# tkkiran/Robust-Conditional-GAN

Measured on AMD Instinct MI355X. Metric: images/sec G+D train step (CIFAR-10 RCGAN bs=64), higher is better.
Workload: dtype bf16

## Files before the change

include/rcgan_hip.h:

```cpp
#ifndef RCGAN_HIP_H
#define RCGAN_HIP_H

#include <stddef.h>
#include <stdint.h>

#ifdef __cplusplus
extern "C" {
#endif

#define RCGAN_OK 0
#define RCGAN_EINVALID_ARG (-1)
#define RCGAN_EUNSUPPORTED_SHAPE (-2)
#define RCGAN_EWORKSPACE_TOO_SMALL (-3)
#define RCGAN_EHIP (-4)
#define RCGAN_ERCCL (-5)

#define RCGAN_F32 0
#define RCGAN_BF16 1
#define RCGAN_F16 2

#define RCGAN_ACT_NONE 0
#define RCGAN_ACT_RELU 1
#define RCGAN_ACT_LRELU 2
#define RCGAN_ACT_TANH 3
// ... 137 lines not shown
int rcgan_bn_bwd(rcgan_ctx* ctx, int n, int rows_per_sample, int c, int n_labels, int dtype,
                 const void* x, const void* y, const void* dy, const int32_t* labels,
                 const float* gamma, const float* mean, const float* rstd, int act,
                 void* dx, int accumulate_dx, float* dgamma, float* dbeta, int accumulate, void* ws, size_t ws_bytes);
int rcgan_bn_bwd2(rcgan_ctx* ctx, int n, int rows_per_sample, int c, int n_labels, int dtype, const void* x, const void* y,
                  const void* dy, const int32_t* labels, const float* gamma, const float* beta, const float* mean, const float* rstd,
                  int act, void* dx, int accumulate_dx, float* dgamma, float* dbeta, int accumulate, void* ws, size_t ws_bytes);
int rcgan_bn_infer(rcgan_ctx* ctx, int rows, int c, int dtype, const void* x, const float* gamma,
                   const float* beta, const float* moving_mean, const float* moving_var, float eps,
                   int act, void* y);
int rcgan_bn_infer_bwd(rcgan_ctx* ctx, int rows, int c, int dtype, const void* y, const void* dy, const float* gamma,
                       const float* moving_var, float eps, int act, void* dx, int accumulate);

typedef struct rcgan_sn_item {
  const float* w;
  float* u;
  float* sigma;
  float* save;
  int k, c, update;
} rcgan_sn_item;
size_t rcgan_sn_save_floats(int k, int c);
int rcgan_sn_power_iter(rcgan_ctx* ctx, const rcgan_sn_item* items, int n_items);
typedef struct rcgan_sn_bwd_item {
  const float* w; const float* dwbar; float* dw; float* save ; int k, c, accumulate;
} rcgan_sn_bwd_item;
int rcgan_sn_bwd(rcgan_ctx* ctx, const rcgan_sn_bwd_item* items, int n_items);
typedef struct rcgan_sn_adam {
  float* w; float* g; float* m; float* v; size_t count;
  float* hyper;
  float beta1, beta2, eps, clip, grad_scale;
  int n_ranges; const size_t* ranges;
} rcgan_sn_adam;
int rcgan_sn_bwd_adam(rcgan_ctx* ctx, const rcgan_sn_bwd_item* items, int n_items, const rcgan_sn_adam* opt);

int rcgan_act_fwd(rcgan_ctx* ctx, size_t count, int dtype, int act, const void* x, void* y);
int rcgan_act_bwd(rcgan_ctx* ctx, size_t count, int dtype, int act, const void* x_or_y, const void* dy,
                  void* dx, int accumulate);
int rcgan_add(rcgan_ctx* ctx, size_t count, int dtype, const void* a, const void* b, void* y);
int rcgan_axpby(rcgan_ctx* ctx, size_t count, int dtype, float alpha, const void* a, float beta, void* y);
int rcgan_cast(rcgan_ctx* ctx, size_t count, int src_dtype, const void* src, int dst_dtype, void* dst);
int rcgan_meanpool2_fwd(rcgan_ctx* ctx, int n, int h, int w, int c, int dtype, const void* x, void* y);
int rcgan_meanpool2_bwd(rcgan_ctx* ctx, int n, int h, int w, int c, int dtype, const void* dy, void* dx, int accumulate);
int rcgan_upsample2_fwd(rcgan_ctx* ctx, int n, int h, int w, int c, int dtype, const void* x, void* y);
int rcgan_upsample2_bwd(rcgan_ctx* ctx, int n, int h, int w, int c, int dtype, const void* dy, void* dx, int accumulate);
int rcgan_pad_channels(rcgan_ctx* ctx, size_t rows, int c, int before, int after, int dtype, const void* x, void* y);
int rcgan_concat_channels_fwd(rcgan_ctx* ctx, int n, int hw, int c1, int c2, int dtype, const void* x,
                              const float* yb, void* y);
int rcgan_concat_channels_bwd(rcgan_ctx* ctx, int n, int hw, int c1, int c2, int dtype, const void* dy, void* dx);
int rcgan_tile_rows_fwd(rcgan_ctx* ctx, size_t count, int reps, int dtype, const void* x, void* y);
int rcgan_tile_rows_bwd(rcgan_ctx* ctx, size_t count, int reps, int dtype, const void* dy, void* dx, int accumulate);
int rcgan_transpose_f32(rcgan_ctx* ctx, int rows, int cols, const float* x, float* y, int accumulate);
int rcgan_preprocess_cifar(rcgan_ctx* ctx, int n, const int32_t* images_chw, const float* noise_chw,
                           int dtype, void* y_nhwc);

int rcgan_rng_fill(rcgan_ctx* ctx, size_t count, int dtype, int kind, float lo, float hi, uint64_t seed,
                   void* state, void* y);

int rcgan_act_meanhw_fwd(rcgan_ctx* ctx, int n, int hw, int c, int dtype, int act, const void* x, float* feat);
int rcgan_act_meanhw_bwd(rcgan_ctx* ctx, int n, int hw, int c, int dtype, int act, const void* x,
                         const float* dfeat, void* dx);
int rcgan_gather_rows(rcgan_ctx* ctx, int n, int d, const float* table, const int32_t* idx, float* out);
int rcgan_scatter_add_rows(rcgan_ctx* ctx, int n, int d, int v, const float* src, const int32_t* idx,
                           float* table_grad, int accumulate);
int rcgan_proj_logit_fwd(rcgan_ctx* ctx, int n, int d, const float* feat, const float* psi, const float* emb,
                         float* logit);
int rcgan_proj_logit_bwd(rcgan_ctx* ctx, int n, int d, const float* feat, const float* emb, const float* dlogit,
// ... 114 lines not shown
```

robust-conditional-gan_amd/_lib.py:

```python
import ctypes as C
import os

_HERE = os.path.dirname(os.path.abspath(__file__))
LIB_PATH = os.environ.get("RCGAN_LIB_PATH") or os.path.join(_HERE, "librcgan_hip.so")
LIB_PATH_F16 = os.environ.get("RCGAN_LIB_PATH_F16") or os.path.join(_HERE, "librcgan_hip_f16.so")

F32, BF16, F16 = 0, 1, 2
ACT_NONE, ACT_RELU, ACT_LRELU, ACT_TANH, ACT_SIGMOID = 0, 1, 2, 3, 4
CONV_IN_UPSAMPLE2X, CONV_IN_RELU, CONV_ACCUMULATE, CONV_FORCE_DIRECT, CONV_OUT_MEANPOOL2, CONV_RESID_UPSAMPLE2X = 1, 2, 4, 8, 16, 32
LOSS_HINGE_REAL, LOSS_HINGE_FAKE, LOSS_NEG_MEAN, LOSS_CE_ONES, LOSS_CE_ZEROS = 0, 1, 2, 3, 4
QUERY_TR_READ = 0
F32_PRECISION_HIGHEST, F32_PRECISION_HIGH = 0, 1
F32_PRECISIONS = {"highest": F32_PRECISION_HIGHEST, "high": F32_PRECISION_HIGH}

RCGAN_EHIP, RCGAN_ERCCL = -4, -5
EINVALID_ARG, EUNSUPPORTED_SHAPE = -1, -2
ERRORS = {-1: "RCGAN_EINVALID_ARG", -2: "RCGAN_EUNSUPPORTED_SHAPE", -3: "RCGAN_EWORKSPACE_TOO_SMALL",
          -4: "RCGAN_EHIP", -5: "RCGAN_ERCCL"}


def source_hash():
    import glob
    import hashlib
    h = hashlib.sha256()
# ... 109 lines not shown
    "rcgan_conv2d_fwd_bn": (I, [P, DP, P, P, P, P, I, P, P, P, P, P, I]),
    "rcgan_conv2d_fwd_bn_residual": (I, [P, DP, P, P, P, P, P, I, P, P, P, P, P, I]),
    "rcgan_conv_fused_pool_ok": (I, [DP]),
    "rcgan_conv_resid_up_ok": (I, [DP]),
    "rcgan_conv_wgrad_pool_ok": (I, [DP]),
    "rcgan_conv2d_fwd_residual": (I, [P, DP, P, P, P, P, P]),
    "rcgan_conv2d_bwd_data": (I, [P, DP, P, P, P, P, P, SZ]),
    "rcgan_conv2d_bwd_data_residual": (I, [P, DP, P, P, P, P, P, P, SZ]),
    "rcgan_conv2d_bwd_weight": (I, [P, DP, P, P, P, P, I, P, SZ]),
    "rcgan_conv2d_bwd_weight_group": (I, [P, I, P, P, P, P, P, I, P, SZ]),
    "rcgan_deconv2d_fwd": (I, [P, DP, P, P, P, P]),
    "rcgan_deconv2d_bwd_data": (I, [P, DP, P, P, P]),
    "rcgan_deconv2d_bwd_data_cols": (I, [P, DP, P, P, P, I]),
    "rcgan_deconv2d_bwd_weight": (I, [P, DP, P, P, P, P, I, P, SZ]),
    "rcgan_deconv2d_bwd_weight_concat_bytes": (SZ, [DP, I]),
    "rcgan_deconv2d_bwd_weight_concat": (I, [P, DP, P, P, I, P, P, P, I, P, SZ]),
    "rcgan_linear_fwd": (I, [P, I, I, I, I, P, P, P, P, P]),
    "rcgan_linear_bwd_data": (I, [P, I, I, I, I, P, P, P, P, I]),
    "rcgan_linear_bwd_weight": (I, [P, I, I, I, I, P, P, P, P, I, P, SZ]),
    "rcgan_linear_workspace_bytes": (SZ, [I, I, I]),
    "rcgan_bn_workspace_bytes": (SZ, [I, I]),
    "rcgan_bn_workspace_bytes_labels": (SZ, [I, I, I]),
    "rcgan_bn_stats": (I, [P, I, I, I, P, F, P, P, P, P, F, P, SZ]),
    "rcgan_bn_apply_fwd": (I, [P, I, I, I, I, I, P, P, P, P, P, P, I, P, P, SZ]),
    "rcgan_bn_fwd_segments": (I, [P, I, I, I, I, I, I, P, P, P, P, F, I, P, P, P, P, SZ]),
    "rcgan_bn_bwd": (I, [P, I, I, I, I, I, P, P, P, P, P, P, P, I, P, I, P, P, I, P, SZ]),
    "rcgan_bn_bwd2": (I, [P, I, I, I, I, I, P, P, P, P, P, P, P, P, I, P, I, P, P, I, P, SZ]),
    "rcgan_bn_infer": (I, [P, I, I, I, P, P, P, P, P, F, I, P]),
    "rcgan_bn_infer_bwd": (I, [P, I, I, I, P, P, P, P, F, I, P, I]),
    "rcgan_sn_save_floats": (SZ, [I, I]),
    "rcgan_sn_power_iter": (I, [P, C.POINTER(SnItem), I]),
    "rcgan_sn_bwd": (I, [P, C.POINTER(SnBwdItem), I]),
    "rcgan_sn_bwd_adam": (I, [P, C.POINTER(SnBwdItem), I, C.POINTER(SnAdam)]),
    "rcgan_act_fwd": (I, [P, SZ, I, I, P, P]),
    "rcgan_act_bwd": (I, [P, SZ, I, I, P, P, P, I]),
    "rcgan_add": (I, [P, SZ, I, P, P, P]),
    "rcgan_axpby": (I, [P, SZ, I, F, P, F, P]),
    "rcgan_cast": (I, [P, SZ, I, P, I, P]),
    "rcgan_meanpool2_fwd": (I, [P, I, I, I, I, I, P, P]),
    "rcgan_meanpool2_bwd": (I, [P, I, I, I, I, I, P, P, I]),
    "rcgan_upsample2_fwd": (I, [P, I, I, I, I, I, P, P]),
    "rcgan_upsample2_bwd": (I, [P, I, I, I, I, I, P, P, I]),
    "rcgan_pad_channels": (I, [P, SZ, I, I, I, I, P, P]),
    "rcgan_concat_channels_fwd": (I, [P, I, I, I, I, I, P, P, P]),
    "rcgan_concat_channels_bwd": (I, [P, I, I, I, I, I, P, P]),
    "rcgan_tile_rows_fwd": (I, [P, SZ, I, I, P, P]),
    "rcgan_tile_rows_bwd": (I, [P, SZ, I, I, P, P, I]),
    "rcgan_transpose_f32": (I, [P, I, I, P, P, I]),
    "rcgan_preprocess_cifar": (I, [P, I, P, P, I, P]),
    "rcgan_rng_fill": (I, [P, SZ, I, I, F, F, C.c_uint64, P, P]),
    "rcgan_act_meanhw_fwd": (I, [P, I, I, I, I, I, P, P]),
    "rcgan_act_meanhw_bwd": (I, [P, I, I, I, I, I, P, P, P]),
    "rcgan_gather_rows": (I, [P, I, I, P, P, P]),
    "rcgan_scatter_add_rows": (I, [P, I, I, I, P, P, P, I]),
    "rcgan_proj_logit_fwd": (I, [P, I, I, P, P, P, P]),
    "rcgan_proj_logit_bwd": (I, [P, I, I, P, P, P, P, P, P, I]),
    "rcgan_proj_logit_all_fwd": (I, [P, I, I, I, P, P, P, P]),
    "rcgan_proj_logit_all_bwd": (I, [P, I, I, I, P, P, P, P, P, P, I]),
    "rcgan_loss_fwd_bwd": (I, [P, I, I, I, P, P, F, P, P, P]),
    "rcgan_bce_onehot_fwd_bwd": (I, [P, I, I, P, P, F, P, P]),
    "rcgan_dtrunk": (I, [P, I, I, P, P, P, P, P]),
    "rcgan_dtrunk_pooled": (I, [P, I, I, P, P, P, P, P, P, P, P]),
    "rcgan_dtrunk_prepare": (I, [P, P, P]),
    "rcgan_conv_rf_ok": (I, [C.POINTER(ConvDesc)]),
    "rcgan_conv_rf_fragment_bytes": (SZ, [C.POINTER(ConvDesc)]),
    "rcgan_conv_rf_prepare": (I, [P, I, C.POINTER(ConvDesc), P, P]),
# ... 70 lines not shown
```

robust-conditional-gan_amd/cifar.py:

```python
import ctypes as C
import os

import warnings

import numpy as np
import torch

from . import _lib as L
from . import ops as O
from .ops_cifar import NO_OPS, Conv2D, Linear, cond_batchnorm, embed_y, spectral_normed_weight
from .runtime import DT, Context, ParamGroup, check_f32_matmul_precision
from .variables import Graph, scoped, variable_scope

Z_DIM = 128
DIM_G = 128
DIM_D = 128
VOCAB_SIZE = 10
EMBEDDING_DIM = 300
IMG_SIZE = 32
IMG_DIM = 3
OUTPUT_DIM = 3072
N_CRITIC = 5
GEN_BS_MULTIPLE = 2
ALGORITHMS = ("rcgan", "rcgan-u", "biased", "unbiased")
# ... 874 lines not shown
            self.PD.version += 1
            return
        self._optimise_or_publish(steps)

    def _critic_graph_ok(self):
        return (self.critic_graph and self.fused_tail and self._fakes_left == N_CRITIC and self._rides_inputs() and self._slice_mirror == 0)

    def critic_steps(self, batches, iteration=None):
        it = self.iteration if iteration is None else iteration
        packed = isinstance(batches, torch.Tensor)
        assert (batches.shape[0] if packed else len(batches)) == N_CRITIC
        if not self._critic_graph_ok():
            for k in range(N_CRITIC):
                if packed:
                    self.set_feed("d", batches[k])
                else:
                    self.feed_host("d", **batches[k])
                self.d_step(iteration=it)
            return
        ctx = self.ctx
        if packed:
            src = batches.reshape(-1)
            assert src.is_cuda and src.dtype == torch.int32 and src.is_contiguous() and src.numel() == self.feed["d5"].numel()
            ctx.check(ctx.lib.rcgan_copy_words(ctx.h, src.numel(), C.c_void_p(src.data_ptr()), C.c_void_p(self.feed["d5"].data_ptr())))
        else:
            self.feed_host("d5", _steps=batches)
        self._refresh_generator_filters()
        lr = self.lr * lr_decay(it)
        self._pre_step([(self.PD, lr)])
        self._join_gf()

        def body():
            fused = True
            for k in range(N_CRITIC):
                saved = {n: self.inp[n] for n in self._d_slot_views[k]}
                self.inp.update(self._d_slot_views[k])
                try:
                    fused = self._d_body(True) and fused
                finally:
                    self.inp.update(saved)
            self._tail_fused["d5"] = fused
        self._run("d5", body)
        assert self._tail_fused.get("d5", False), "critic_steps: a step's last launch did not apply the update"
        self._fakes_left = 0
        self.PD.t += N_CRITIC
        self.PD._dev_hyper = (float(lr), self.PD.t)
        self.PD.version += 1

    def g_step(self, iteration=None):
        it = self.iteration if iteration is None else iteration
        self._fakes_left = 0
        self._join_gf()
        self._refresh_generator_filters()
        steps = [(self.PG, self.lr * lr_decay(it))]
        if self.PC is not None:
            steps.append((self.PC, self.lr * self.confuse_multiplier * (lr_decay(it) if self.confuse_lr_decay else 1.0)))
        self._pre_step(steps)
        self._run("g", self._g_body)
        self._optimise_or_publish(steps)
        self._refresh_generator_filters()

    def _optimise(self, steps):
        ctx = self.ctx
        if not self.dynamic_ls:
            for grp, lr in steps:
                grp.t += 1
                grp.set_hyper(lr, grp.t)
                grp.adam(0.0, 0.9, grad_scale=1.0 / (self.world * self.loss_scale))
            return
        for grp, lr in steps:
            grp.t += 1
            grp.finite_check(self.ls_state)
        for grp, lr in steps:
# ... 141 lines not shown
```

robust-conditional-gan_amd/csrc/sn.hip:

```cpp
#include <algorithm>
#include <utility>
#include <vector>

#include "common.h"

#define SN_MAX_K 4096
#define SN_MAX_C 1024
#define SN_BATCH 24
#define SN_EPS 1e-12f
#define SN_RB 32
#define SN_NT 256
#define SN_NW (SN_NT / 64)
#define SN_MAX_CHUNKS (SN_MAX_K / SN_RB)

struct SnLayout {
  float *a, *v, *dv, *b, *u2, *uin, *db, *s, *pb, *pgw, *pdva;
  int chunks;
};
__host__ __device__ inline int sn_chunks(int k) { return (k + SN_RB - 1) / SN_RB; }
__device__ __forceinline__ SnLayout sn_layout(float* save, int k, int c) {
  SnLayout L;
  L.chunks = sn_chunks(k);
  const int kp = (k + 3) & ~3, cp = (c + 3) & ~3;
  L.a = save; L.v = L.a + kp; L.dv = L.v + kp;
  L.b = L.dv + kp; L.u2 = L.b + cp; L.uin = L.u2 + cp; L.db = L.uin + cp;
  L.s = L.db + cp;
  L.pb = L.s + 4;
  L.pgw = L.pb + (long)L.chunks * c;
  L.pdva = L.pgw + L.chunks;
  return L;
}

__device__ __forceinline__ float block_sum_nt(float v, float* red ) {
  v = wave_sum(v);
  __syncthreads();
  if ((threadIdx.x & 63) == 0) red[threadIdx.x >> 6] = v;
  __syncthreads();
  float r = 0.f;
#pragma unroll
  for (int i = 0; i < SN_NW; ++i) r += red[i];
  return r;
}

struct SnBatch { rcgan_sn_item it[SN_BATCH]; unsigned* arrive;  };
struct SnBwdBatch { rcgan_sn_bwd_item it[SN_BATCH]; };

template <bool AGENT> __device__ __forceinline__ void sn_fwd_finish(const rcgan_sn_item& it, float* red);

__global__ __launch_bounds__(SN_NT) void sn_fwd_rows_kernel(SnBatch batch) {
  __shared__ float a_s[SN_RB];
  const rcgan_sn_item it = batch.it[blockIdx.y];
  const int k = it.k, c = it.c;
  const int r0 = blockIdx.x * SN_RB;
  if (r0 >= k) return;
  const int rows = min(SN_RB, k - r0);
  const SnLayout L = sn_layout(it.save, k, c);
  const float* w = it.w + (long)r0 * c;
  const int tid = threadIdx.x, lane = tid & 63, wave = tid >> 6;
  float part[SN_RB / SN_NW];
#pragma unroll
  for (int i = 0; i < SN_RB / SN_NW; ++i) {
    const int r = wave + i * SN_NW;
    float s = 0.f;
    if (r < rows)
      for (int j = lane; j < c; j += 64) s += w[(long)r * c + j] * it.u[j];
    part[i] = s;
  }
#pragma unroll
  for (int i = 0; i < SN_RB / SN_NW; ++i) {
    const int r = wave + i * SN_NW;
    const float s = wave_sum(part[i]);
    if (lane == 0 && r < rows) { a_s[r] = s; __hip_atomic_store(L.a + r0 + r, s, __ATOMIC_RELAXED, __HIP_MEMORY_SCOPE_AGENT); }
  }
  __syncthreads();
  for (int j = tid; j < c; j += SN_NT) {
    float s = 0.f;
#pragma unroll 8
    for (int r = 0; r < rows; ++r) s += a_s[r] * w[(long)r * c + j];
// ... 123 lines not shown
  }
  __syncthreads();
  float gw = 0.f, pa = 0.f;
  float part[SN_RB / SN_NW], av[SN_RB / SN_NW];
#pragma unroll
  for (int i = 0; i < SN_RB / SN_NW; ++i) {
    const int r = wave + i * SN_NW;
    float s = 0.f;
    if (small_c) {
      const float q0 = lane < c ? q_s[lane] : 0.f, q1 = lane + 64 < c ? q_s[lane + 64] : 0.f;
      s = wr[i][0] * q0 + wr[i][1] * q1;
      gw += gr[i][0] * wr[i][0] + gr[i][1] * wr[i][1];
    } else if (r < rows) {
      for (int j = lane; j < c; j += 64) {
        const float wv = w[(long)r * c + j];
        s += wv * q_s[j];
        gw += g[(long)r * c + j] * wv;
      }
    }
    part[i] = s;
    av[i] = (lane == 0 && r < rows) ? L.a[r0 + r] : 0.f;
  }
#pragma unroll
  for (int i = 0; i < SN_RB / SN_NW; ++i) {
    const int r = wave + i * SN_NW;
    const float s = wave_sum(part[i]);
    if (lane == 0 && r < rows) { L.dv[r0 + r] = s; pa += s * av[i]; }
  }
  gw = block_sum_nt(gw, red);
  pa = block_sum_nt(lane == 0 ? pa : 0.f, red);
  if (tid == 0) { L.pgw[blockIdx.x] = gw; L.pdva[blockIdx.x] = pa; }
}

template <bool ADAM>
__global__ __launch_bounds__(SN_NT) void sn_bwd_p2_kernel(SnBwdBatch batch, int n_items, SnAdam ad) {
  __shared__ float da_s[SN_RB];
  __shared__ float v_s[SN_RB];
  __shared__ float red[SN_NW];
  const int tid = threadIdx.x;
  float alpha = 0.f, omb1 = 0.f, omb2 = 0.f;
  if (ADAM) {
    const float lr = ad.hyper[0], t = ad.hyper[1];
    alpha = lr * sqrtf(1.f - powf(ad.beta2, t)) / (1.f - powf(ad.beta1, t));
    omb1 = 1.f - ad.beta1;
    omb2 = 1.f - ad.beta2;
    if ((int)blockIdx.y >= n_items) {
      for (int rg = 0; rg < ad.n_ranges; ++rg)
        for (unsigned o = ad.lo[rg] + blockIdx.x * SN_NT + tid; o < ad.hi[rg]; o += gridDim.x * SN_NT) {
          float m = ad.m_base[o], v = ad.v_base[o], wv = ad.w_base[o];
          sn_adam_elem(ad.g_base[o], m, v, wv, alpha, omb1, omb2, ad.eps, ad.clip, ad.grad_scale);
          ad.m_base[o] = m; ad.v_base[o] = v; ad.w_base[o] = wv;
        }
      return;
    }
  }
  const rcgan_sn_bwd_item it = batch.it[blockIdx.y];
  const int k = it.k, c = it.c;
  const int r0 = blockIdx.x * SN_RB;
  if (r0 >= k) return;
  const int rows = min(SN_RB, k - r0);
  const SnLayout L = sn_layout(it.save, k, c);
  const float* g = it.dwbar + (long)r0 * c;
  float* dw = it.dw + (long)r0 * c;
  constexpr int PF = SN_RB * 128 / 4 / SN_NT;
  const bool pf = (c & 3) == 0 && c <= 128;
  const long aoff = ADAM ? (long)(dw - ad.g_base) : 0;
  float4 pg[PF], pd[PF], pm[PF], pv[PF], pw[PF];
  if (pf) {
    const int n4 = rows * (c >> 2);
#pragma unroll
    for (int e = 0; e < PF; ++e) {
      const int i = tid + e * SN_NT;
      const bool ok = i < n4;
      const float4 z4 = make_float4(0.f, 0.f, 0.f, 0.f);
      pg[e] = ok ? ((const float4*)g)[i] : z4;
      pd[e] = (ok && it.accumulate) ? ((const float4*)dw)[i] : z4;
      if (ADAM) {
        pm[e] = ok ? ((const float4*)(ad.m_base + aoff))[i] : z4;
        pv[e] = ok ? ((const float4*)(ad.v_base + aoff))[i] : z4;
        pw[e] = ok ? ((const float4*)(ad.w_base + aoff))[i] : z4;
      }
    }
  }
  const float na = L.s[0], sigma = L.s[2];
  float gw = 0.f, pa = 0.f;
  for (int q = tid; q < L.chunks; q += SN_NT) { gw += L.pgw[q]; pa += L.pdva[q]; }
  gw = block_sum_nt(gw, red);
  pa = block_sum_nt(pa, red);
  const float dsigma = -gw / (sigma * sigma);
  const float dva = dsigma * pa;
  const float inv_na = 1.f / (na + SN_EPS);
  const float coef_a = dva / (na * (na + SN_EPS) * (na + SN_EPS));
  if (tid < rows) {
    da_s[tid] = dsigma * L.dv[r0 + tid] * inv_na - L.a[r0 + tid] * coef_a;
    v_s[tid] = dsigma * L.v[r0 + tid];
  }
  __syncthreads();
  const float inv_sigma = 1.f / sigma;
  if (pf) {
    const int c4 = c >> 2, n4 = rows * c4;
    float4* dw4 = (float4*)dw;
    const float4* q4 = (const float4*)L.db;
    const float4* u4 = (const float4*)L.uin;
#pragma unroll
    for (int e = 0; e < PF; ++e) {
      const int i = tid + e * SN_NT;
      if (i >= n4) break;
      const int r = i / c4, j = i - r * c4;
      const float4 gv = pg[e], d = q4[j], u = u4[j];
      const float vr = v_s[r], ar = da_s[r];
      float4 o;
      o.x = gv.x * inv_sigma + vr * d.x + ar * u.x;
      o.y = gv.y * inv_sigma + vr * d.y + ar * u.y;
      o.z = gv.z * inv_sigma + vr * d.z + ar * u.z;
      o.w = gv.w * inv_sigma + vr * d.w + ar * u.w;
      if (it.accumulate) { o.x += pd[e].x; o.y += pd[e].y; o.z += pd[e].z; o.w += pd[e].w; }
      dw4[i] = o;
      if (ADAM) {
        float4 m = pm[e], v = pv[e], wv = pw[e];
        sn_adam_elem(o.x, m.x, v.x, wv.x, alpha, omb1, omb2, ad.eps, ad.clip, ad.grad_scale);
        sn_adam_elem(o.y, m.y, v.y, wv.y, alpha, omb1, omb2, ad.eps, ad.clip, ad.grad_scale);
        sn_adam_elem(o.z, m.z, v.z, wv.z, alpha, omb1, omb2, ad.eps, ad.clip, ad.grad_scale);
        sn_adam_elem(o.w, m.w, v.w, wv.w, alpha, omb1, omb2, ad.eps, ad.clip, ad.grad_scale);
        ((float4*)(ad.m_base + aoff))[i] = m;
        ((float4*)(ad.v_base + aoff))[i] = v;
        ((float4*)(ad.w_base + aoff))[i] = wv;
      }
    }
  } else if ((c & 3) == 0) {
    const int c4 = c >> 2;
    const float4* g4 = (const float4*)g;
    float4* dw4 = (float4*)dw;
    const float4* q4 = (const float4*)L.db;
    const float4* u4 = (const float4*)L.uin;
    for (int i = tid; i < rows * c4; i += SN_NT) {
      const int r = i / c4, j = i - r * c4;
      const float4 gv = g4[i], d = q4[j], u = u4[j];
      const float vr = v_s[r], ar = da_s[r];
      float4 o;
      o.x = gv.x * inv_sigma + vr * d.x + ar * u.x;
      o.y = gv.y * inv_sigma + vr * d.y + ar * u.y;
      o.z = gv.z * inv_sigma + vr * d.z + ar * u.z;
      o.w = gv.w * inv_sigma + vr * d.w + ar * u.w;
      if (it.accumulate) { float4 p = dw4[i]; o.x += p.x; o.y += p.y; o.z += p.z; o.w += p.w; }
      dw4[i] = o;
      if (ADAM) {
        float4* m4 = (float4*)(ad.m_base + aoff) + i;
        float4* vv4 = (float4*)(ad.v_base + aoff) + i;
        float4* w4 = (float4*)(ad.w_base + aoff) + i;
        float4 m = *m4, v = *vv4, wv = *w4;
        sn_adam_elem(o.x, m.x, v.x, wv.x, alpha, omb1, omb2, ad.eps, ad.clip, ad.grad_scale);
        sn_adam_elem(o.y, m.y, v.y, wv.y, alpha, omb1, omb2, ad.eps, ad.clip, ad.grad_scale);
        sn_adam_elem(o.z, m.z, v.z, wv.z, alpha, omb1, omb2, ad.eps, ad.clip, ad.grad_scale);
        sn_adam_elem(o.w, m.w, v.w, wv.w, alpha, omb1, omb2, ad.eps, ad.clip, ad.grad_scale);
        *m4 = m; *vv4 = v; *w4 = wv;
      }
    }
  } else {
    for (int i = tid; i < rows * c; i += SN_NT) {
      const int r = i / c, j = i - r * c;
      float o = g[i] * inv_sigma + v_s[r] * L.db[j] + da_s[r] * L.uin[j];
      if (it.accumulate) o += dw[i];
      dw[i] = o;
      if (ADAM) {
        float m = ad.m_base[aoff + i], v = ad.v_base[aoff + i], wv = ad.w_base[aoff + i];
        sn_adam_elem(o, m, v, wv, alpha, omb1, omb2, ad.eps, ad.clip, ad.grad_scale);
        ad.m_base[aoff + i] = m; ad.v_base[aoff + i] = v; ad.w_base[aoff + i] = wv;
      }
    }
  }
}

extern "C" {

size_t rcgan_sn_save_floats(int k, int c) {
  const size_t kp = ((size_t)k + 3) & ~(size_t)3, cp = ((size_t)c + 3) & ~(size_t)3;
  return 3 * kp + 4 * cp + 4 + (size_t)sn_chunks(k) * ((size_t)c + 2);
}

int rcgan_sn_power_iter(rcgan_ctx* ctx, const rcgan_sn_item* items, int n_items) {
  for (int base = 0; base < n_items; base += SN_BATCH) {
    SnBatch b;
    int n = n_items - base < SN_BATCH ? n_items - base : SN_BATCH;
    int maxk = 1;
    for (int i = 0; i < n; ++i) {
      b.it[i] = items[base + i];
      if (b.it[i].k > SN_MAX_K || b.it[i].c > SN_MAX_C || b.it[i].k < 1 || b.it[i].c < 1)
        RC_FAIL(ctx, RCGAN_EUNSUPPORTED_SHAPE, "sn weight [%d,%d]", b.it[i].k, b.it[i].c);
      if (b.it[i].k > maxk) maxk = b.it[i].k;
    }
    static const int fused = [] { const char* e = getenv("RCGAN_SN_FUSED_FINISH"); return e ? atoi(e) : 0; }();
    b.arrive = fused ? ctx->tree_counters() : nullptr;
    hipLaunchKernelGGL(sn_fwd_rows_kernel, dim3(sn_chunks(maxk), n), dim3(SN_NT), 0, ctx->stream, b);
    RC_LAUNCH_CHECK(ctx);
    if (!fused) {
      hipLaunchKernelGGL(sn_fwd_finish_kernel, dim3(n), dim3(SN_NT), 0, ctx->stream, b);
      RC_LAUNCH_CHECK(ctx);
    }
  }
  return RCGAN_OK;
}

static int sn_bwd_launch(rcgan_ctx* ctx, const rcgan_sn_bwd_item* items, int n_items, const rcgan_sn_adam* opt) {
  for (int base = 0; base < n_items; base += SN_BATCH) {
    SnBwdBatch b;
    int n = n_items - base < SN_BATCH ? n_items - base : SN_BATCH;
    int maxk = 1;
    for (int i = 0; i < n; ++i) {
      b.it[i] = items[base + i];
      if (b.it[i].k > SN_MAX_K || b.it[i].c > SN_MAX_C || b.it[i].k < 1 || b.it[i].c < 1)
        RC_FAIL(ctx, RCGAN_EUNSUPPORTED_SHAPE, "sn weight [%d,%d]", b.it[i].k, b.it[i].c);
      if (b.it[i].k > maxk) maxk = b.it[i].k;
    }
    const dim3 grid(sn_chunks(maxk), n);
    hipLaunchKernelGGL(sn_bwd_p1_kernel, grid, dim3(SN_NT), 0, ctx->stream, b, (opt && base == 0) ? opt->hyper : (float*)nullptr);
    RC_LAUNCH_CHECK(ctx);
    SnAdam ad = {};
    if (opt) {
      const bool last = base + n >= n_items;
      ad.w_base = opt->w; ad.m_base = opt->m; ad.v_base = opt->v; ad.g_base = opt->g; ad.hyper = opt->hyper;
      ad.beta1 = opt->beta1; ad.beta2 = opt->beta2; ad.eps = opt->eps; ad.clip = opt->clip; ad.grad_scale = opt->grad_scale;
      ad.riders = last ? 1 : 0;
      ad.n_ranges = last ? opt->n_ranges : 0;
      for (int r = 0; r < ad.n_ranges; ++r) { ad.lo[r] = (unsigned)opt->ranges[2 * r]; ad.hi[r] = (unsigned)opt->ranges[2 * r + 1]; }
      hipLaunchKernelGGL(sn_bwd_p2_kernel<true>, dim3(grid.x, n + (last ? 1 : 0)), dim3(SN_NT), 0, ctx->stream, b, n, ad);
    } else {
      hipLaunchKernelGGL(sn_bwd_p2_kernel<false>, grid, dim3(SN_NT), 0, ctx->stream, b, n, ad);
    }
    RC_LAUNCH_CHECK(ctx);
  }
  return RCGAN_OK;
}

int rcgan_sn_bwd(rcgan_ctx* ctx, const rcgan_sn_bwd_item* items, int n_items) { return sn_bwd_launch(ctx, items, n_items, nullptr); }

int rcgan_sn_bwd_adam(rcgan_ctx* ctx, const rcgan_sn_bwd_item* items, int n_items, const rcgan_sn_adam* opt) {
  RC_REQUIRE(ctx, items && n_items >= 1 && opt && opt->w && opt->g && opt->m && opt->v && opt->hyper, "null argument");
  RC_REQUIRE(ctx, opt->count < (1ull << 32) && opt->n_ranges >= 0 && opt->n_ranges <= SN_MAX_RANGES && (opt->n_ranges == 0 || opt->ranges),
             "%zu parameters, %d ranges (at most %d)", opt->count, opt->n_ranges, SN_MAX_RANGES);
  std::vector<std::pair<size_t, size_t>> iv;
  for (int i = 0; i < n_items; ++i) {
    const size_t sz = (size_t)items[i].k * items[i].c;
    RC_REQUIRE(ctx, items[i].w >= opt->w && items[i].w + sz <= opt->w + opt->count, "item %d: w outside the slab", i);
    RC_REQUIRE(ctx, items[i].dw - opt->g == items[i].w - opt->w, "item %d: dw and w at different slab offsets", i);
    auto a16 = [](const void* p) { return ((size_t)p & 15) == 0; };
    RC_REQUIRE(ctx, items[i].c % 4 != 0 || ((items[i].w - opt->w) % 4 == 0 && a16(items[i].w) && a16(items[i].dwbar) && a16(items[i].dw) &&
                                            a16(items[i].save) && a16(opt->m) && a16(opt->v)),
               "item %d ([%d,%d]): c %% 4 == 0 needs a slab offset that is a multiple of 4 floats and 16-byte aligned w, dwbar, dw, save, m, v",
               i, items[i].k, items[i].c);
    iv.push_back({(size_t)(items[i].w - opt->w), (size_t)(items[i].w - opt->w) + sz});
  }
  for (int r = 0; r < opt->n_ranges; ++r) {
    RC_REQUIRE(ctx, opt->ranges[2 * r] <= opt->ranges[2 * r + 1] && opt->ranges[2 * r + 1] <= opt->count, "range %d outside the slab", r);
    iv.push_back({opt->ranges[2 * r], opt->ranges[2 * r + 1]});
  }
  std::sort(iv.begin(), iv.end());
  size_t at = 0;
  for (auto& p : iv) {
    if (p.first == p.second) continue;
    RC_REQUIRE(ctx, p.first == at, "items and ranges must tile the slab: gap or overlap at float offset %zu (next piece starts at %zu)", at, p.first);
    at = p.second;
  }
  RC_REQUIRE(ctx, at == opt->count, "items and ranges cover %zu of %zu parameters", at, opt->count);
  return sn_bwd_launch(ctx, items, n_items, opt);
}

}
```

robust-conditional-gan_amd/ops.py:

```python
import ctypes as C
import os

import torch

from . import _lib as L
from .runtime import DT


def _p(t):
    return C.c_void_p(t.ptr) if t is not None else None


def same_pad(n, k, s):
    out = -(-n // s)
    tot = max((out - 1) * s + k - n, 0)
    return out, tot // 2


def zeros_like_grad(ctx, t):
    g = ctx.empty(t.shape, t.dtype)
    ctx.check(ctx.lib.rcgan_fill_f32(ctx.h, (g.nbytes + 3) // 4, g.ptr, 0.0))
    return g


# ... 143 lines not shown
    tp = tf = None
    if trunk:
        tdesc = L.ConvDesc(1, 8, 8, 128, 128, 3, 3, 1, ctx.act_dtype, L.CONV_IN_RELU)
        tp = (C.c_void_p * 8)(*[w.prepared(tdesc).ptr for w in trunk])
        nb = ctx.lib.rcgan_dtrunk_fragment_bytes()
        tf = DT(ctx.arena.alloc(nb), (nb,), "u8", ctx.arena.buf)
    n = len(rf)
    descs = (L.ConvDesc * max(n, 1))(*[d for _, d in rf])
    preps = (C.c_void_p * max(n, 1))(*[w.prepared(d).ptr for w, d in rf])
    frags = []
    for w, d in rf:
        nb = ctx.lib.rcgan_conv_rf_fragment_bytes(C.byref(d))
        w.rf_frag = DT(ctx.arena.alloc(nb), (nb,), "u8", ctx.arena.buf)
        frags.append(w.rf_frag.ptr)
    ctx.check(ctx.lib.rcgan_fragments_prepare(ctx.h, tp, _p(tf), n, descs, preps, (C.c_void_p * max(n, 1))(*frags)))
    return tf


def spectral_norm_batch(ctx, entries):
    n = len(entries)
    if n == 0:
        return []
    items = (L.SnItem * n)()
    weights = []
    saves = []
    for i, (param, u, update) in enumerate(entries):
        c = param.shape[-1]
        k = param.size // c
        sigma = ctx.empty((1,), L.F32)
        save = ctx.empty((ctx.lib.rcgan_sn_save_floats(k, c),), L.F32)
        items[i] = L.SnItem(param.ptr, u.ptr, sigma.ptr, save.ptr, k, c, 1 if update else 0)
        weights.append(Weight(ctx, param, sigma))
        saves.append((save, k, c))
    ctx.check(ctx.lib.rcgan_sn_power_iter(ctx.h, items, n))
    if ctx.recording:
        req = [w for w in weights if w.param.req]
        total = sum((w.param.size + 63) // 64 * 64 for w in req)
        if total and all(w.param.group is not None and w.param.group.sn_scratch and w.param.group.zero_epoch == ctx.epoch for w in req):
            for w in req:
                w.dwbar = w.param.group.dwbar(w.param.name)
        elif total:
            base = ctx.arena.alloc(total * 4)
            ctx.check(ctx.lib.rcgan_fill_f32(ctx.h, total, base, 0.0))
            off = 0
            for w in req:
                w.dwbar = DT(base + off * 4, w.param.shape, L.F32, ctx.arena.buf)
                off += (w.param.size + 63) // 64 * 64

    done = set()

    def bw(only=None):
        ctx.flush_wgrads()
        todo = [(i, w, s) for i, (w, s) in enumerate(zip(weights, saves))
                if i not in done and w.dwbar is not None and w.param.req and (only is None or only(w.param.name))]
        if not todo:
            return
        bi = (L.SnBwdItem * len(todo))()
        for j, (i, w, (save, k, c)) in enumerate(todo):
            bi[j] = L.SnBwdItem(w.param.ptr, w.dwbar.ptr, w.param.grad.ptr, save.ptr, k, c, 1)
            done.add(i)
        fa = getattr(ctx, "sn_adam", None)
        ranges = None
        if fa is not None and not fa.get("done") and len(todo) == len(weights) and all(w.param.group is fa["group"] for _, w, _ in todo):
            grp = fa["group"]
            cover = sorted((grp.offsets[w.param.name], grp.offsets[w.param.name] + w.param.size) for _, w, _ in todo)
            ranges, at = [], 0
            for lo, hi in cover:
                if lo > at:
                    ranges += [at, lo]
                at = hi
            if at < grp.count:
                ranges += [at, grp.count]
            if len(ranges) // 2 > L.SN_MAX_RANGES or grp.count >= 1 << 32:
                ranges = None
        if ranges is not None:
            ra = (C.c_size_t * max(len(ranges), 1))(*ranges)
            opt = L.SnAdam(grp.value.data_ptr(), grp.grad.data_ptr(), grp.m.data_ptr(), grp.v.data_ptr(), grp.count, grp.hyper.data_ptr(),
                           fa["beta1"], fa["beta2"], fa.get("eps", 1e-8), fa.get("clip", 0.0), fa["grad_scale"], len(ranges) // 2, ra)
            ctx.check(ctx.lib.rcgan_sn_bwd_adam(ctx.h, bi, len(todo), C.byref(opt)))
            fa["done"] = True
            return
        ctx.check(ctx.lib.rcgan_sn_bwd(ctx.h, bi, len(todo)))
    if any(p.req for p, _, _ in entries):
        ctx.record(bw)
        ctx.sn_partial.append(bw)
    return weights


FUSE_BN_STATS = os.environ.get("RCGAN_FUSE_BN_STATS", "0") == "1"


def conv2d(ctx, x, weight, bias, k, stride=1, in_up=False, in_relu=False, accumulate_into=None, force_direct=False,
           residual=None, residual_up=False, want_stats=False):
    if isinstance(x, BnPending):
        pend = x
        n, hs, ws_, cin = pend.shape
        cout = weight.param.shape[-1]
        assert weight.param.shape == (k, k, cin, cout), (weight.param.shape, (k, k, cin, cout))
        bh, bw = (hs * 2, ws_ * 2) if in_up else (hs, ws_)
        bflags = (L.CONV_IN_UPSAMPLE2X if in_up else 0) | (L.CONV_RESID_UPSAMPLE2X if (residual is not None and residual_up) else 0)
        bdesc = L.ConvDesc(n, bh, bw, cin, cout, k, k, stride, pend.dtype, bflags)
        if (not in_relu and accumulate_into is None and not force_direct and not ctx.recording and stride == 1
                and pend.act in (L.ACT_NONE, L.ACT_RELU) and ctx.lib.rcgan_conv_bn_in_ok(C.byref(bdesc))
                and (residual is None or (residual.shape == ((n, bh // 2, bw // 2, cout) if residual_up else (n, bh, bw, cout))
                                          and (not residual_up or ctx.lib.rcgan_conv_resid_up_ok(C.byref(bdesc)))))):
            y = ctx.empty((n, bh, bw, cout), pend.dtype)
            pdesc = L.ConvDesc(n, bh, bw, cin, cout, k, k, stride, pend.dtype, L.CONV_IN_UPSAMPLE2X if in_up else 0)
            rc = ctx.lib.rcgan_conv2d_fwd_bn_residual(ctx.h, C.byref(bdesc), _p(pend.x), _p(weight.prepared(pdesc)), _p(bias), _p(residual), _p(y),
                                                      pend.segments, _p(pend.labels), _p(pend.gamma), _p(pend.beta), _p(pend.mean),
                                                      _p(pend.rstd), pend.act)
            if rc == 0:
                return y
# ... 831 lines not shown
```

robust-conditional-gan_amd/runtime.py:

```python
import ctypes as C

import os

import numpy as np
import torch

from . import _lib as L

ALIGN = 256


def _np_dtype(code):
    return np.float32 if code == L.F32 else np.uint16


class DT:
    __slots__ = ("ptr", "shape", "dtype", "base", "grad", "req", "name", "frozen", "group", "tile_stats", "pooled", "pool_grad", "concat_src", "concat_labels")

    def __init__(self, ptr, shape, dtype, base=None, name=None):
        self.ptr = int(ptr)
        self.shape = tuple(int(s) for s in shape)
        self.dtype = dtype
        self.base = base
        self.grad = None
# ... 69 lines not shown
        raise ValueError("Unknown f32_matmul_precision %r: one of %s" % (precision, ", ".join(sorted(L.F32_PRECISIONS))))
    if precision != "highest" and dtype != "f32":
        raise ValueError("f32_matmul_precision=%r needs dtype='f32' (got %r)" % (precision, dtype))
    return precision


class Context:

    def __init__(self, device=0, dtype="bf16", arena_bytes=6 << 30, ws_bytes=1 << 30):
        if not torch.cuda.is_available():
            raise RuntimeError("no HIP device visible: the RCGAN engine has no CPU fallback")
        if dtype in ("f16", "fp16", L.F16):
            self.act_dtype, self.lib = L.F16, L.load("f16")
        else:
            self.act_dtype, self.lib = (L.BF16 if dtype in ("bf16", L.BF16) else L.F32), L.load()
        self.device = torch.device("cuda", device)
        torch.cuda.set_device(self.device)
        self.stream = torch.cuda.Stream(device=self.device)
        h = C.c_void_p()
        rc = self.lib.rcgan_create(C.byref(h), device, C.c_void_p(self.stream.cuda_stream))
        if rc != 0:
            raise L.RcganError(rc, "rcgan_create failed")
        self.h = h
        self.arena = Arena(arena_bytes, self.device)
        self.ws = torch.empty(int(ws_bytes), dtype=torch.uint8, device=self.device)
        self.ws_ptr, self.ws_bytes = self.ws.data_ptr(), int(ws_bytes)
        self.epoch = 0
        self.overlap = os.environ.get("RCGAN_OVERLAP", "0") == "1"
        self.ws2 = torch.empty(int(ws_bytes), dtype=torch.uint8, device=self.device) if self.overlap else None
        self.ws2_ptr = self.ws2.data_ptr() if self.overlap else 0
        self.tape = []
        self.sn_partial = []
        self.pending_wgrads = []
        self.group_wgrads = os.environ.get("RCGAN_GROUP_WGRAD", "1") == "1"
        self.recording = True
        self.capturing = False
        self._keep = []
        self.check(self.lib.rcgan_selftest(self.h))
        self.uses_tr_read = self.lib.rcgan_query(self.h, L.QUERY_TR_READ)

    def check(self, rc):
        if rc != 0:
            raise L.RcganError(rc, self.lib.rcgan_last_error(self.h).decode())

    def close(self):
        for c in getattr(self, "also_close", []):
            c.close()
        self.also_close = []
        if self.h is not None:
            self.lib.rcgan_destroy(self.h)
            self.h = None

    def empty(self, shape, dtype=None, name=None):
        dtype = self.act_dtype if dtype is None else dtype
        n = 1
        for s in shape:
            n *= int(s)
        isz = 4 if dtype in (L.F32, "i32") else 2
        return DT(self.arena.alloc(max(n, 1) * isz), shape, dtype, self.arena.buf, name)

    def persistent(self, shape, dtype=L.F32, fill=None):
        tdt = {L.F32: torch.float32, L.BF16: torch.bfloat16, L.F16: torch.float16, "i32": torch.int32}[dtype]
        t = torch.empty(tuple(int(s) for s in shape) or (1,), dtype=tdt, device=self.device)
        if fill is not None:
            with torch.cuda.stream(self.stream):
                t.fill_(fill)
# ... 247 lines not shown
```

Before: 61650.

## Fold next critic step's spectral-norm row pass into the SN backward Adam kernel

```diff
diff --git a/include/rcgan_hip.h b/include/rcgan_hip.h
--- a/include/rcgan_hip.h
+++ b/include/rcgan_hip.h
@@ -193,6 +193,8 @@
   int n_ranges; const size_t* ranges;
 } rcgan_sn_adam;
 int rcgan_sn_bwd_adam(rcgan_ctx* ctx, const rcgan_sn_bwd_item* items, int n_items, const rcgan_sn_adam* opt);
+int rcgan_sn_bwd_adam_rows(rcgan_ctx* ctx, const rcgan_sn_bwd_item* items, int n_items, const rcgan_sn_adam* opt, const rcgan_sn_item* next);
+int rcgan_sn_power_iter_finish(rcgan_ctx* ctx, const rcgan_sn_item* items, int n_items);
 
 int rcgan_act_fwd(rcgan_ctx* ctx, size_t count, int dtype, int act, const void* x, void* y);
 int rcgan_act_bwd(rcgan_ctx* ctx, size_t count, int dtype, int act, const void* x_or_y, const void* dy,
diff --git a/robust-conditional-gan_amd/_lib.py b/robust-conditional-gan_amd/_lib.py
--- a/robust-conditional-gan_amd/_lib.py
+++ b/robust-conditional-gan_amd/_lib.py
@@ -165,6 +165,8 @@
     "rcgan_sn_power_iter": (I, [P, C.POINTER(SnItem), I]),
     "rcgan_sn_bwd": (I, [P, C.POINTER(SnBwdItem), I]),
     "rcgan_sn_bwd_adam": (I, [P, C.POINTER(SnBwdItem), I, C.POINTER(SnAdam)]),
+    "rcgan_sn_bwd_adam_rows": (I, [P, C.POINTER(SnBwdItem), I, C.POINTER(SnAdam), C.POINTER(SnItem)]),
+    "rcgan_sn_power_iter_finish": (I, [P, C.POINTER(SnItem), I]),
     "rcgan_act_fwd": (I, [P, SZ, I, I, P, P]),
     "rcgan_act_bwd": (I, [P, SZ, I, I, P, P, P, I]),
     "rcgan_add": (I, [P, SZ, I, P, P, P]),
diff --git a/robust-conditional-gan_amd/cifar.py b/robust-conditional-gan_amd/cifar.py
--- a/robust-conditional-gan_amd/cifar.py
+++ b/robust-conditional-gan_amd/cifar.py
@@ -930,13 +930,19 @@
 
         def body():
             fused = True
-            for k in range(N_CRITIC):
-                saved = {n: self.inp[n] for n in self._d_slot_views[k]}
-                self.inp.update(self._d_slot_views[k])
-                try:
-                    fused = self._d_body(True) and fused
-                finally:
-                    self.inp.update(saved)
+            ctx.sn_fold = {"next": False, "rows": None}
+            try:
+                for k in range(N_CRITIC):
+                    saved = {n: self.inp[n] for n in self._d_slot_views[k]}
+                    self.inp.update(self._d_slot_views[k])
+                    ctx.sn_fold["next"] = k + 1 < N_CRITIC
+                    try:
+                        fused = self._d_body(True) and fused
+                    finally:
+                        self.inp.update(saved)
+                assert ctx.sn_fold["rows"] is None, "critic_steps: a folded row pass was left without its finish"
+            finally:
+                ctx.sn_fold = None
             self._tail_fused["d5"] = fused
         self._run("d5", body)
         assert self._tail_fused.get("d5", False), "critic_steps: a step's last launch did not apply the update"
diff --git a/robust-conditional-gan_amd/csrc/sn.hip b/robust-conditional-gan_amd/csrc/sn.hip
--- a/robust-conditional-gan_amd/csrc/sn.hip
+++ b/robust-conditional-gan_amd/csrc/sn.hip
@@ -44,6 +44,8 @@
 
 struct SnBatch { rcgan_sn_item it[SN_BATCH]; unsigned* arrive;  };
 struct SnBwdBatch { rcgan_sn_bwd_item it[SN_BATCH]; };
+#define SN_FOLD_MAX_C 256
+struct SnRows { const float* u[SN_BATCH]; float* save[SN_BATCH]; };
 
 template <bool AGENT> __device__ __forceinline__ void sn_fwd_finish(const rcgan_sn_item& it, float* red);
 
@@ -233,8 +235,10 @@
   if (tid == 0) { L.pgw[blockIdx.x] = gw; L.pdva[blockIdx.x] = pa; }
 }
 
-template <bool ADAM>
-__global__ __launch_bounds__(SN_NT) void sn_bwd_p2_kernel(SnBwdBatch batch, int n_items, SnAdam ad) {
+template <bool ADAM, bool ROWS>
+__global__ __launch_bounds__(SN_NT) void sn_bwd_p2_kernel(SnBwdBatch batch, int n_items, SnAdam ad, SnRows rw) {
+  static_assert(ADAM || !ROWS, "the row pass reads the rows the optimiser has just written");
+  __shared__ __attribute__((aligned(16))) float w_s[ROWS ? SN_RB * SN_FOLD_MAX_C : 4];
   __shared__ float da_s[SN_RB];
   __shared__ float v_s[SN_RB];
   __shared__ float red[SN_NW];
@@ -282,6 +286,13 @@
         pw[e] = ok ? ((const float4*)(ad.w_base + aoff))[i] : z4;
       }
     }
+  }
+  const bool u_pf = ROWS && c <= 128;
+  float un0 = 0.f, un1 = 0.f;
+  if (u_pf) {
+    const int lane = tid & 63;
+    un0 = lane < c ? rw.u[blockIdx.y][lane] : 0.f;
+    un1 = lane + 64 < c ? rw.u[blockIdx.y][lane + 64] : 0.f;
   }
   const float na = L.s[0], sigma = L.s[2];
   float gw = 0.f, pa = 0.f;
@@ -326,6 +337,7 @@
         ((float4*)(ad.m_base + aoff))[i] = m;
         ((float4*)(ad.v_base + aoff))[i] = v;
         ((float4*)(ad.w_base + aoff))[i] = wv;
+        if (ROWS) ((float4*)w_s)[i] = wv;
       }
     }
   } else if ((c & 3) == 0) {
@@ -355,6 +367,7 @@
         sn_adam_elem(o.z, m.z, v.z, wv.z, alpha, omb1, omb2, ad.eps, ad.clip, ad.grad_scale);
         sn_adam_elem(o.w, m.w, v.w, wv.w, alpha, omb1, omb2, ad.eps, ad.clip, ad.grad_scale);
         *m4 = m; *vv4 = v; *w4 = wv;
+        if (ROWS) ((float4*)w_s)[i] = wv;
       }
     }
   } else {
@@ -367,7 +380,43 @@
         float m = ad.m_base[aoff + i], v = ad.v_base[aoff + i], wv = ad.w_base[aoff + i];
         sn_adam_elem(o, m, v, wv, alpha, omb1, omb2, ad.eps, ad.clip, ad.grad_scale);
         ad.m_base[aoff + i] = m; ad.v_base[aoff + i] = v; ad.w_base[aoff + i] = wv;
-      }
+        if (ROWS) w_s[i] = wv;
+      }
+    }
+  }
+  if (ROWS) {
+    const float* u = rw.u[blockIdx.y];
+    const SnLayout N = sn_layout(rw.save[blockIdx.y], k, c);
+    const int lane = tid & 63, wave = tid >> 6;
+    float* a_s = da_s;
+    __syncthreads();
+    float part[SN_RB / SN_NW];
+#pragma unroll
+    for (int i = 0; i < SN_RB / SN_NW; ++i) {
+      const int r = wave + i * SN_NW;
+      float s = 0.f;
+      if (r < rows) {
+        if (u_pf) {
+          if (lane < c) s += w_s[r * c + lane] * un0;
+          if (lane + 64 < c) s += w_s[r * c + lane + 64] * un1;
+        } else {
+          for (int j = lane; j < c; j += 64) s += w_s[r * c + j] * u[j];
+        }
+      }
+      part[i] = s;
+    }
+#pragma unroll
+    for (int i = 0; i < SN_RB / SN_NW; ++i) {
+      const int r = wave + i * SN_NW;
+      const float s = wave_sum(part[i]);
+      if (lane == 0 && r < rows) { a_s[r] = s; __hip_atomic_store(N.a + r0 + r, s, __ATOMIC_RELAXED, __HIP_MEMORY_SCOPE_AGENT); }
+    }
+    __syncthreads();
+    for (int j = tid; j < c; j += SN_NT) {
+      float s = 0.f;
+#pragma unroll 8
+      for (int r = 0; r < rows; ++r) s += a_s[r] * w_s[r * c + j];
+      __hip_atomic_store(N.pb + (long)blockIdx.x * c + j, s, __ATOMIC_RELAXED, __HIP_MEMORY_SCOPE_AGENT);
     }
   }
 }
@@ -379,7 +428,7 @@
   return 3 * kp + 4 * cp + 4 + (size_t)sn_chunks(k) * ((size_t)c + 2);
 }
 
-int rcgan_sn_power_iter(rcgan_ctx* ctx, const rcgan_sn_item* items, int n_items) {
+static int sn_fwd_launch(rcgan_ctx* ctx, const rcgan_sn_item* items, int n_items, bool rows, bool finish) {
   for (int base = 0; base < n_items; base += SN_BATCH) {
     SnBatch b;
     int n = n_items - base < SN_BATCH ? n_items - base : SN_BATCH;
@@ -391,10 +440,12 @@
       if (b.it[i].k > maxk) maxk = b.it[i].k;
     }
     static const int fused = [] { const char* e = getenv("RCGAN_SN_FUSED_FINISH"); return e ? atoi(e) : 0; }();
-    b.arrive = fused ? ctx->tree_counters() : nullptr;
-    hipLaunchKernelGGL(sn_fwd_rows_kernel, dim3(sn_chunks(maxk), n), dim3(SN_NT), 0, ctx->stream, b);
-    RC_LAUNCH_CHECK(ctx);
-    if (!fused) {
+    b.arrive = (fused && rows && finish) ? ctx->tree_counters() : nullptr;
+    if (rows) {
+      hipLaunchKernelGGL(sn_fwd_rows_kernel, dim3(sn_chunks(maxk), n), dim3(SN_NT), 0, ctx->stream, b);
+      RC_LAUNCH_CHECK(ctx);
+    }
+    if (finish && b.arrive == nullptr) {
       hipLaunchKernelGGL(sn_fwd_finish_kernel, dim3(n), dim3(SN_NT), 0, ctx->stream, b);
       RC_LAUNCH_CHECK(ctx);
     }
@@ -402,16 +453,24 @@
   return RCGAN_OK;
 }
 
-static int sn_bwd_launch(rcgan_ctx* ctx, const rcgan_sn_bwd_item* items, int n_items, const rcgan_sn_adam* opt) {
+int rcgan_sn_power_iter(rcgan_ctx* ctx, const rcgan_sn_item* items, int n_items) { return sn_fwd_launch(ctx, items, n_items, true, true); }
+
+int rcgan_sn_power_iter_finish(rcgan_ctx* ctx, const rcgan_sn_item* items, int n_items) {
+  RC_REQUIRE(ctx, items && n_items >= 1, "null argument");
+  return sn_fwd_launch(ctx, items, n_items, false, true);
+}
+
+static int sn_bwd_launch(rcgan_ctx* ctx, const rcgan_sn_bwd_item* items, int n_items, const rcgan_sn_adam* opt, const rcgan_sn_item* next = nullptr) {
   for (int base = 0; base < n_items; base += SN_BATCH) {
     SnBwdBatch b;
     int n = n_items - base < SN_BATCH ? n_items - base : SN_BATCH;
-    int maxk = 1;
+    int maxk = 1, maxc = 1;
     for (int i = 0; i < n; ++i) {
       b.it[i] = items[base + i];
       if (b.it[i].k > SN_MAX_K || b.it[i].c > SN_MAX_C || b.it[i].k < 1 || b.it[i].c < 1)
         RC_FAIL(ctx, RCGAN_EUNSUPPORTED_SHAPE, "sn weight [%d,%d]", b.it[i].k, b.it[i].c);
       if (b.it[i].k > maxk) maxk = b.it[i].k;
+      if (b.it[i].c > maxc) maxc = b.it[i].c;
     }
     const dim3 grid(sn_chunks(maxk), n);
     hipLaunchKernelGGL(sn_bwd_p1_kernel, grid, dim3(SN_NT), 0, ctx->stream, b, (opt && base == 0) ? opt->hyper : (float*)nullptr);
@@ -424,18 +483,30 @@
       ad.riders = last ? 1 : 0;
       ad.n_ranges = last ? opt->n_ranges : 0;
       for (int r = 0; r < ad.n_ranges; ++r) { ad.lo[r] = (unsigned)opt->ranges[2 * r]; ad.hi[r] = (unsigned)opt->ranges[2 * r + 1]; }
-      hipLaunchKernelGGL(sn_bwd_p2_kernel<true>, dim3(grid.x, n + (last ? 1 : 0)), dim3(SN_NT), 0, ctx->stream, b, n, ad);
+      SnRows rw = {};
+      const bool fold = next != nullptr && maxc <= SN_FOLD_MAX_C;
+      if (fold) {
+        for (int i = 0; i < n; ++i) { rw.u[i] = next[base + i].u; rw.save[i] = next[base + i].save; }
+        hipLaunchKernelGGL((sn_bwd_p2_kernel<true, true>), dim3(grid.x, n + (last ? 1 : 0)), dim3(SN_NT), 0, ctx->stream, b, n, ad, rw);
+      } else {
+        hipLaunchKernelGGL((sn_bwd_p2_kernel<true, false>), dim3(grid.x, n + (last ? 1 : 0)), dim3(SN_NT), 0, ctx->stream, b, n, ad, rw);
+      }
+      RC_LAUNCH_CHECK(ctx);
+      if (next != nullptr && !fold) {
+        const int rc = sn_fwd_launch(ctx, next + base, n, true, false);
+        if (rc != RCGAN_OK) return rc;
+      }
     } else {
-      hipLaunchKernelGGL(sn_bwd_p2_kernel<false>, grid, dim3(SN_NT), 0, ctx->stream, b, n, ad);
-    }
-    RC_LAUNCH_CHECK(ctx);
+      hipLaunchKernelGGL((sn_bwd_p2_kernel<false, false>), grid, dim3(SN_NT), 0, ctx->stream, b, n, ad, SnRows{});
+      RC_LAUNCH_CHECK(ctx);
+    }
   }
   return RCGAN_OK;
 }
 
 int rcgan_sn_bwd(rcgan_ctx* ctx, const rcgan_sn_bwd_item* items, int n_items) { return sn_bwd_launch(ctx, items, n_items, nullptr); }
 
-int rcgan_sn_bwd_adam(rcgan_ctx* ctx, const rcgan_sn_bwd_item* items, int n_items, const rcgan_sn_adam* opt) {
+static int sn_bwd_adam_checked(rcgan_ctx* ctx, const rcgan_sn_bwd_item* items, int n_items, const rcgan_sn_adam* opt, const rcgan_sn_item* next) {
   RC_REQUIRE(ctx, items && n_items >= 1 && opt && opt->w && opt->g && opt->m && opt->v && opt->hyper, "null argument");
   RC_REQUIRE(ctx, opt->count < (1ull << 32) && opt->n_ranges >= 0 && opt->n_ranges <= SN_MAX_RANGES && (opt->n_ranges == 0 || opt->ranges),
              "%zu parameters, %d ranges (at most %d)", opt->count, opt->n_ranges, SN_MAX_RANGES);
@@ -463,7 +534,19 @@
     at = p.second;
   }
   RC_REQUIRE(ctx, at == opt->count, "items and ranges cover %zu of %zu parameters", at, opt->count);
-  return sn_bwd_launch(ctx, items, n_items, opt);
-}
-
-}
+  return sn_bwd_launch(ctx, items, n_items, opt, next);
+}
+
+int rcgan_sn_bwd_adam(rcgan_ctx* ctx, const rcgan_sn_bwd_item* items, int n_items, const rcgan_sn_adam* opt) {
+  return sn_bwd_adam_checked(ctx, items, n_items, opt, nullptr);
+}
+
+int rcgan_sn_bwd_adam_rows(rcgan_ctx* ctx, const rcgan_sn_bwd_item* items, int n_items, const rcgan_sn_adam* opt, const rcgan_sn_item* next) {
+  RC_REQUIRE(ctx, items && n_items >= 1 && next, "null argument");
+  for (int i = 0; i < n_items; ++i)
+    RC_REQUIRE(ctx, next[i].w == items[i].w && next[i].k == items[i].k && next[i].c == items[i].c && next[i].u && next[i].save,
+               "item %d: the next power iteration must be of the same weight ([%d,%d]) with u and save set", i, items[i].k, items[i].c);
+  return sn_bwd_adam_checked(ctx, items, n_items, opt, next);
+}
+
+}
diff --git a/robust-conditional-gan_amd/ops.py b/robust-conditional-gan_amd/ops.py
--- a/robust-conditional-gan_amd/ops.py
+++ b/robust-conditional-gan_amd/ops.py
@@ -199,7 +199,15 @@
         items[i] = L.SnItem(param.ptr, u.ptr, sigma.ptr, save.ptr, k, c, 1 if update else 0)
         weights.append(Weight(ctx, param, sigma))
         saves.append((save, k, c))
-    ctx.check(ctx.lib.rcgan_sn_power_iter(ctx.h, items, n))
+    fold = getattr(ctx, "sn_fold", None)
+    if fold is not None and fold.get("rows") is not None:
+        key = [(it.w, it.u, it.sigma, it.save, it.k, it.c, it.update) for it in items]
+        if key != fold["rows"]:
+            raise RuntimeError("spectral_norm_batch: the folded row pass of the previous step was taken for other items than this call's")
+        fold["rows"] = None
+        ctx.check(ctx.lib.rcgan_sn_power_iter_finish(ctx.h, items, n))
+    else:
+        ctx.check(ctx.lib.rcgan_sn_power_iter(ctx.h, items, n))
     if ctx.recording:
         req = [w for w in weights if w.param.req]
         total = sum((w.param.size + 63) // 64 * 64 for w in req)
@@ -244,7 +252,12 @@
             ra = (C.c_size_t * max(len(ranges), 1))(*ranges)
             opt = L.SnAdam(grp.value.data_ptr(), grp.grad.data_ptr(), grp.m.data_ptr(), grp.v.data_ptr(), grp.count, grp.hyper.data_ptr(),
                            fa["beta1"], fa["beta2"], fa.get("eps", 1e-8), fa.get("clip", 0.0), fa["grad_scale"], len(ranges) // 2, ra)
-            ctx.check(ctx.lib.rcgan_sn_bwd_adam(ctx.h, bi, len(todo), C.byref(opt)))
+            fold = getattr(ctx, "sn_fold", None)
+            if fold is not None and fold.get("next") and len(todo) == n:
+                ctx.check(ctx.lib.rcgan_sn_bwd_adam_rows(ctx.h, bi, len(todo), C.byref(opt), items))
+                fold["rows"] = [(it.w, it.u, it.sigma, it.save, it.k, it.c, it.update) for it in items]
+            else:
+                ctx.check(ctx.lib.rcgan_sn_bwd_adam(ctx.h, bi, len(todo), C.byref(opt)))
             fa["done"] = True
             return
         ctx.check(ctx.lib.rcgan_sn_bwd(ctx.h, bi, len(todo)))
diff --git a/robust-conditional-gan_amd/runtime.py b/robust-conditional-gan_amd/runtime.py
--- a/robust-conditional-gan_amd/runtime.py
+++ b/robust-conditional-gan_amd/runtime.py
@@ -125,6 +125,7 @@
         self.tape = []
         self.sn_partial = []
         self.pending_wgrads = []
+        self.sn_fold = None
         self.group_wgrads = os.environ.get("RCGAN_GROUP_WGRAD", "1") == "1"
         self.recording = True
         self.capturing = False
```

Result: no change. 61950 (median of 6 runs) (+0.5%).
